# ykevinc/pocket-tts

Measured on AMD Instinct MI355X. Metric: audio-sec/wall-sec (RTF) per GPU at batch=32 + p50 first-chunk latency, higher is better.
Workload: dtype f32; 1 GPU; b6369a24 batch=32 concurrent 10 s utterances per GPU (125 frames, voice prompt 125 frames, 40 text tokens), lsd_decode_steps=1 (BASELINE configs[2]); global_batch=32, utterance_frames=125, jobs=37, prompt_frames=125, parallelism=replicas x1

## Files before the change

pocket-tts_amd/csrc/engine.cpp:

```cpp
#include "engine.h"

#include <hip/hip_ext.h>

#include <algorithm>
#include <array>
#include <cstdlib>
#include <cmath>
#include <cstring>
#include <mutex>

namespace ptts {

namespace {
std::mutex& voice_mu() {
  static std::mutex m;
  return m;
}

int pick_splits(int M, int N, int K) {
  const int tiles = ((N + 31) / 32) * ((M + 31) / 32);
  const int chunks = K / 32;
  int s = std::max(1, 768 / std::max(1, tiles));
  s = std::min(s, std::max(1, chunks / 4));
  return std::min(s, 16);
// ... 48 lines not shown
  PTTS_REQUIRE(!(cfg.fp8_gemm && cfg.weight_quant != QUANT_NONE), "fp8_gemm and weight_quant are exclusive");
  fp8_ = cfg.fp8_gemm;
  PTTS_REQUIRE(cfg.back_frames >= 0 && cfg.back_frames <= NFR_MAX && !(cfg.back_frames & (cfg.back_frames - 1)),
               "back_frames must be 0, 1, 2, 4 or 8");
  nfr_ = cfg.pipeline && cfg.back_frames >= 2 ? cfg.back_frames : 1;
  PTTS_REQUIRE(cfg.back_mfma >= PTTS_BACK_F32 && cfg.back_mfma <= PTTS_BACK_F32X6, "unknown back_mfma mode");
  back_mfma_ = cfg.back_mfma;
  nhb_ = nfr_ > 1 ? 3 * nfr_ : 3;
  int ndev = 0;
  PTTS_HIP(hipGetDeviceCount(&ndev));
  PTTS_REQUIRE(dev_ >= 0 && dev_ < ndev, "HIP device ordinal out of range");
  PTTS_HIP(hipSetDevice(dev_));
  PTTS_HIP(hipStreamCreateWithFlags(&stream_, hipStreamNonBlocking));

  L_ = pack_weights(nullptr, nullptr);
  if (cfg.weight_blob) {
    blob_ = (float*)cfg.weight_blob;
    own_blob_ = false;
  } else {
    blob_ = dalloc(L_.total);
  }

  const int B = max_slots_;
  kv_layer_ = (long)2 * NH * max_ctx_ * 64;
  kv_slot_ = kv_layer_ * NL;
  kv_ = dalloc((size_t)kv_slot_ * B);
  ring_layer_ = (long)2 * MNH * RING * 64;
  ring_slot_ = ring_layer_ * MNL;
  ring_ = dalloc((size_t)ring_slot_ * B);
  fpos_ = (int*)dalloc(B);
  mpos_ = (int*)dalloc(B);
  st_ = (SlotState*)dalloc((sizeof(SlotState) * B + 3) / 4);
  lat_in_ = dalloc((size_t)B * LDIM);
  cur_ = dalloc((size_t)B * LDIM);
  qprev_ = dalloc((size_t)(1 + NFR_MAX) * B * MD);
  qcur_ = qprev_ + (size_t)B * MD;
  eos_ = dalloc(B);
  static_assert(sizeof(FrameFlags) == 2 * sizeof(float), "FrameFlags packs into two floats");
  meta_floats_ = (size_t)B * (LDIM + 1 + 2);
  const size_t mstride = (meta_floats_ + 31) / 32 * 32;
  if (nfr_ > 1)
    for (int p = 0; p < nhb_ / nfr_; ++p) {
      const size_t n = (size_t)B * nfr_ * FRAME + nfr_ * mstride;
      pcmp_[p] = dalloc(n);
      PTTS_HIP(hipHostMalloc((void**)&h_pcmp_[p], sizeof(float) * n, hipHostMallocDefault));
    }
  for (int q = 0; q < NHB; ++q) {
    meta_[q] = nfr_ > 1 && q < nhb_ ? pcmp_[q / nfr_] + (size_t)B * nfr_ * FRAME + (q % nfr_) * mstride
                                    : dalloc(meta_floats_);
    lat_out_[q] = meta_[q];
    flags_[q] = (FrameFlags*)(meta_[q] + (size_t)B * LDIM);
    eos_out_[q] = meta_[q] + (size_t)B * (LDIM + 2);
    pcm_[q] = dalloc((size_t)B * FRAME);
  }
  fin_side_ = dalloc((size_t)B * (nfr_ * FRAME / RESBLOCK_FIN_TT) * 2);
  PTTS_HIP(hipHostMalloc((void**)&h_act_, sizeof(SlotState) * B, hipHostMallocDefault));
  mpcap_ = (size_t)nfr_ * std::max({(size_t)8 * B * UP * MD, (size_t)4 * B * UP * RATIOS[0] * (MD / 2)});
  mpartial_ = dalloc(mpcap_);

  const int hT[8] = {16, 16, 96, 96, 480, 480, 1920, 1920};
  const int hC[8] = {512, 512, 256, 256, 128, 128, 64, 64};
  const int hP[8] = {6, 1, 2, 1, 2, 1, 2, 2};
  for (int i = 0; i < 8; ++i) {
    hist_T_[i] = hT[i];
    hist_C_[i] = hC[i];
    hist_P_[i] = hP[i];
    hist_[i] = dalloc((size_t)B * hP[i] * hC[i]);
  }

  const int R = std::max(B, PREFILL);
  x_ = dalloc((size_t)R * D);
  h_ = dalloc((size_t)R * D);
  q_ = dalloc((size_t)R * D);
  o_ = dalloc((size_t)R * D);
  u_ = dalloc((size_t)R * FF);
  pcap_ = std::max({(size_t)4 << 20, (size_t)2 * B * UP * 3 * MD, (size_t)PREFILL * FF});
  partial_ = dalloc(pcap_);
  tslab_ = dalloc(TAIL_CAP);
  tickets_ = (int*)dalloc(TICKETS);
  fbm_.x = x_, fbm_.h = h_, fbm_.q = q_, fbm_.o = o_, fbm_.u = u_, fbm_.partial = partial_;
  fbm_.pcap = pcap_, fbm_.tslab = tslab_, fbm_.tail_cap = (long)TAIL_CAP, fbm_.tickets = tickets_;
  fbm_.kv = KvStore{kv_, kv_slot_, max_ctx_};
  fbm_.kv_layer = kv_layer_;
  ids_dev_ = (int*)dalloc(PREFILL);
  rowtab_dev_ = (int*)dalloc(PREFILL);
  ctab_dev_ = (int*)dalloc(PREFILL);
  qrow_dev_ = (int*)dalloc(PREFILL);
  orow_dev_ = (int*)dalloc(PREFILL);
  admit_slots_ = (int*)dalloc(B);
  admit_st_ = (SlotState*)dalloc((sizeof(SlotState) * B + 3) / 4);
  admit_fpos_ = (int*)dalloc(B);
  vpre_ = (const float**)dalloc((sizeof(float*) * B + 3) / 4);
  vlen_ = (int*)dalloc(B);
  slot_voice_.assign(B, nullptr);
  drained_.assign(B, 1);
  admit_call_.assign(B, -1);
  slot_lsd_.assign(B, 0);
  share_voice_ = probe_env("PTTS_NO_SHARED_VOICE") == nullptr;
#ifdef PTTS_PROBES
  if (probe_env("PTTS_STAMPS")) {
    stamp_ring_ = (unsigned long long*)dalloc((size_t)STAMP_CAP * 4);
    stamp_ctr_ = (unsigned*)dalloc(1);
  }
#endif
  if (probe_env("PTTS_BACK_WG_CAP")) back_cap_ = atoi(probe_env("PTTS_BACK_WG_CAP"));
  if (probe_env("PTTS_FRONT_PRIO")) set_front_prio(atoi(probe_env("PTTS_FRONT_PRIO")));
  if (probe_env("PTTS_BACK_PRIO")) set_back_prio(atoi(probe_env("PTTS_BACK_PRIO")));
  if (probe_env("PTTS_FRONT_SKIP")) set_front_skip(atoi(probe_env("PTTS_FRONT_SKIP")));
  ysilu_ = dalloc((size_t)lsd_ * B * FD);
  mods_ = dalloc((size_t)lsd_ * B * NADA);
  xf_ = dalloc((size_t)B * FD);
  hf_ = dalloc((size_t)B * FD);
  uf_ = dalloc((size_t)B * FD);
  PTTS_REQUIRE(hx_floats(B) * 4 < (1ull << 31), "flow-head hand-off regions exceed 2 GB (lsd_decode_steps too large)");
  hx_ = dalloc(hx_floats(B));
  fhm_ = dalloc((size_t)lsd_ * ((B + 15) / 16) * (FDEPTH + 1) * 2 * 16 * FD);
  PTTS_HIP(hipMemset(hx_, 0xFF, hx_floats(B) * 4));
  PTTS_HIP(hipDeviceSynchronize());
  hctr_ = (int*)dalloc(4 * ((B + 15) / 16) + 4);
  herr_ = (int*)dalloc(4);
  const size_t BF = (size_t)B * nfr_;
  mx_ = dalloc(BF * UP * MD);
  mh_ = dalloc(BF * UP * MD);
  mq_ = dalloc(BF * UP * MD);
  mo_ = dalloc(BF * UP * MD);
  mqkv_ = dalloc(BF * UP * 3 * MD);
  mu_ = dalloc(BF * UP * MFF);
  a0_ = dalloc(BF * 16 * 512);
  int T = 16, ch = 512;
  for (int i = 0; i < 3; ++i) {
    T *= RATIOS[i];
    ch /= 2;
    cb_[i] = dalloc(BF * T * ch);
    ce_[i] = dalloc(BF * T * ch);
    cv_[i] = dalloc(BF * T * (ch / 2));
    ca_[i] = dalloc(BF * T * ch);
    trb_[i] = dalloc((size_t)RATIOS[i] * ch);
  }
  temb_ = dalloc((size_t)temb_row0(lsd_ + 1) * FD);
  rope_ = dalloc((size_t)max_ctx_ * 64);
  temb_tmp_ = dalloc((size_t)2 * lsd_ * FD);

  for (int q = 0; q < NHB; ++q) {
    PTTS_HIP(hipHostMalloc((void**)&h_pcm_[q], sizeof(float) * B * FRAME, hipHostMallocDefault));
    if (nfr_ > 1 && q < nhb_)
      h_meta_[q] = h_pcmp_[q / nfr_] + (size_t)B * nfr_ * FRAME + (q % nfr_) * ((meta_floats_ + 31) / 32 * 32);
    else
      PTTS_HIP(hipHostMalloc((void**)&h_meta_[q], sizeof(float) * meta_floats_, hipHostMallocDefault));
    memset(h_meta_[q], 0, sizeof(float) * meta_floats_);
  }
  PTTS_HIP(hipHostMalloc((void**)&h_err_, sizeof(int), hipHostMallocDefault));
  *h_err_ = 0;
  PTTS_HIP(hipHostMalloc((void**)&h_slots_, sizeof(int) * B, hipHostMallocDefault));
  PTTS_HIP(hipHostMalloc((void**)&h_st_, sizeof(SlotState) * B, hipHostMallocDefault));
  PTTS_HIP(hipHostMalloc((void**)&h_fp_, sizeof(int) * B, hipHostMallocDefault));
  PTTS_HIP(hipHostMalloc((void**)&h_ids_, sizeof(int) * PREFILL, hipHostMallocDefault));
  PTTS_HIP(hipHostMalloc((void**)&h_tab_, sizeof(int) * 4 * PREFILL, hipHostMallocDefault));
  PTTS_HIP(hipHostMalloc((void**)&h_vpre_, sizeof(float*) * B, hipHostMallocDefault));
  PTTS_HIP(hipHostMalloc((void**)&h_vlen_, sizeof(int) * B, hipHostMallocDefault));
  memset(h_vpre_, 0, sizeof(float*) * B);
  memset(h_vlen_, 0, sizeof(int) * B);
  PTTS_HIP(hipStreamCreateWithFlags(&stream_be_, hipStreamNonBlocking));
  for (int q = 0; q < NHB; ++q) {
    PTTS_HIP(hipEventCreateWithFlags(&ev_front_[q], hipEventDisableTiming));
    PTTS_HIP(hipEventCreateWithFlags(&ev_back_[q], hipEventDisableTiming));
    PTTS_HIP(hipEventRecord(ev_front_[q], stream_));
    PTTS_HIP(hipEventRecord(ev_back_[q], stream_));
  }
  PTTS_HIP(hipEventCreateWithFlags(&ev_admit_, hipEventDisableTiming));
  PTTS_HIP(hipEventCreateWithFlags(&ev_be_tail_, hipEventDisableTiming));
  PTTS_HIP(hipEventCreateWithFlags(&ev_act_, hipEventDisableTiming));
  for (hipEvent_t& e : ev_call_) PTTS_HIP(hipEventCreateWithFlags(&e, hipEventDisableTiming));
  PTTS_HIP(hipEventRecord(ev_act_, stream_));
  PTTS_HIP(hipEventRecord(ev_admit_, stream_));
  pipeline_ = cfg.pipeline != 0;
  head_resident_ = flow_head_max_resident(dev_);

  if (!cfg.defer_weights) {
    std::unique_ptr<TensorSource> src = cfg.weights_path && cfg.weights_path[0]
                                            ? make_safetensors_source(cfg.weights_path)
                                            : make_synth_source(cfg.synth_seed);
    src = make_quant_source(std::move(src), wq_);
    upload_weights(src.get());
    finalize();
  }
}

Engine::~Engine() {
  (void)hipSetDevice(dev_);
  if (stream_) (void)hipStreamSynchronize(stream_);
  if (stream_be_) (void)hipStreamSynchronize(stream_be_);
  if (stream_pv_) (void)hipStreamSynchronize(stream_pv_);
  if (stream_vc_) (void)hipStreamSynchronize(stream_vc_);
#ifdef PTTS_PROBES
  if (stamp_ring_) {
    unsigned n = 0;
    std::vector<unsigned long long> r((size_t)STAMP_CAP * 2);
    if (hipMemcpy(&n, stamp_ctr_, 4, hipMemcpyDeviceToHost) == hipSuccess &&
        hipMemcpy(r.data(), stamp_ring_, r.size() * 8, hipMemcpyDeviceToHost) == hipSuccess)
      if (FILE* f = fopen(probe_env("PTTS_STAMPS"), "w")) {
        for (int p = 0; p < 2; ++p)
          for (size_t i = 0; i < stamp_names_[p].size(); ++i) fprintf(f, "# %d %zu %s\n", p, i, stamp_names_[p][i].c_str());
        for (unsigned i = 0; i < std::min(n, STAMP_CAP); ++i) fprintf(f, "%llu %llu\n", r[2 * i], r[2 * i + 1]);
        fclose(f);
      }
  }
#endif
  for (int s = 0; s < (int)slot_voice_.size(); ++s) voice_release(s, true);
  for (auto& kv : graphs_) (void)hipGraphExecDestroy(kv.second);
  for (auto& kv : graph_defs_) (void)hipGraphDestroy(kv.second);
  for (auto& kv : pv_graphs_) (void)hipGraphExecDestroy(kv.second);
  for (auto& kv : pv_graph_defs_) (void)hipGraphDestroy(kv.second);
  for (PvEntry& q : pv_q_) {
    if (q.ev) (void)hipEventDestroy(q.ev);
    if (q.h_pcm) (void)hipHostFree(q.h_pcm);
  }
  for (int q = 0; q < NHB; ++q)
    if (ev_pv_read_[q]) (void)hipEventDestroy(ev_pv_read_[q]);
  if (ev_pv_front_) (void)hipEventDestroy(ev_pv_front_);
  if (stream_pv_) (void)hipStreamDestroy(stream_pv_);
  for (int q = 0; q < NHB; ++q) {
    if (ev_front_[q]) (void)hipEventDestroy(ev_front_[q]);
    if (ev_back_[q]) (void)hipEventDestroy(ev_back_[q]);
  }
  if (ev_admit_) (void)hipEventDestroy(ev_admit_);
  if (ev_be_tail_) (void)hipEventDestroy(ev_be_tail_);
  if (ev_act_) (void)hipEventDestroy(ev_act_);
  for (hipEvent_t e : ev_call_)
    if (e) (void)hipEventDestroy(e);
  if (stream_be_) (void)hipStreamDestroy(stream_be_);
  vws_free(vws_);
  for (hipEvent_t e : vws_.ev_up)
    if (e) (void)hipEventDestroy(e);
  if (stream_vc_) (void)hipStreamDestroy(stream_vc_);
  for (void* p : allocs_) (void)hipFree(p);
  for (int q = 0; q < NHB; ++q) {
    if (h_pcm_[q]) (void)hipHostFree(h_pcm_[q]);
    if (h_meta_[q] && !(nfr_ > 1 && q < nhb_)) (void)hipHostFree(h_meta_[q]);
  }
  for (int p = 0; p < NHB / 2; ++p)
    if (h_pcmp_[p]) (void)hipHostFree(h_pcmp_[p]);
  if (h_act_) (void)hipHostFree(h_act_);
  if (h_err_) (void)hipHostFree(h_err_);
  for (void* hp : {(void*)h_slots_, (void*)h_st_, (void*)h_fp_, (void*)h_ids_, (void*)h_tab_, (void*)h_vpre_,
                   (void*)h_vlen_})
    if (hp) (void)hipHostFree(hp);
  if (stream_) (void)hipStreamDestroy(stream_);
}

void Engine::upload_weights(TensorSource* src) {
  std::vector<float> host(L_.total, 0.f);
  pack_weights(src, host.data());
  PTTS_HIP(hipMemcpy(blob_, host.data(), host.size() * sizeof(float), hipMemcpyHostToDevice));
}

void Engine::load_blob(const float* host, size_t n_bytes) {
  PTTS_REQUIRE(n_bytes == L_.total * sizeof(float), "blob size differs from ptts_weight_blob_bytes()");
  PTTS_REQUIRE(!ready_, "engine already finalized");
  PTTS_HIP(hipSetDevice(dev_));
  PTTS_HIP(hipMemcpy(blob_, host, n_bytes, hipMemcpyHostToDevice));
}

const uint32_t* Engine::pack_codes(const float* W, int N, int K, int nj,
                                   const std::function<void(const float*, float*)>& pack) {
  auto it = q8map_.find(W);
  auto it8 = f8map_.find(W);
  if (it == q8map_.end() && it8 == f8map_.end()) return nullptr;
  const size_t n = (size_t)N * K;
  float* tmp = nullptr;
  PTTS_HIP(hipMalloc(&tmp, sizeof(float) * 2 * n));
  void* q = nullptr;
  PTTS_HIP(hipMalloc(&q, n));
  allocs_.push_back(q);
  if (it != q8map_.end()) codes_to_f32(it->second.first, (long)n, tmp, stream_);
  else codes_u8_to_f32(it8->second.first, (long)n, tmp, stream_);
  pack(tmp, tmp + n);
  pack_q8(tmp + n, (long)(n / 4), nj, (uint32_t*)q, stream_);
  PTTS_HIP(hipStreamSynchronize(stream_));
  PTTS_HIP(hipFree(tmp));
  return (const uint32_t*)q;
}

void Engine::derive_gemv() {
  int mask = pipeline_ && nfr_ == 1 ? 2 | 8 | 16 : 31;
  if (probe_env("PTTS_GEMV_MASK")) mask = atoi(probe_env("PTTS_GEMV_MASK"));
  gemv_mask_ = mask;
  struct M {
    const float* w;
    int N, K, bit;
    GemvShape g;
  };
  std::vector<M> mats;
  const GemvShape wide{4, 128};
  const GemvShape outg{1, 32};
  for (int l = 0; l < NL; ++l) {
    const Layout::TL& t = L_.fl[l];
    mats.push_back({W(t.in_proj), 3 * D, D, 1, wide});
    mats.push_back({W(t.out_proj), D, D, 2, outg});
    mats.push_back({W(t.l1), FF, D, 4, wide});
    mats.push_back({W(t.l2), D, FF, 8, GemvShape{1, 64}});
  }
  const GemvShape ada{4, 128};
  mats.push_back({W(L_.ada_w), NADA, FD, 16, ada});
  auto scale_of = [&](const float* w) { return fp8_ ? f8map_.at(w).second : q8map_.at(w).second; };
  if ((mask & 4) && !probe_env("PTTS_NO_FK") && gemv_fk_supported(1, FF, D)) {
    const bool ffn = !probe_env("PTTS_NO_FFN") && ffn_fused_supported(1, D, FF);
    if (ffn) ffn_groups_ = probe_env("PTTS_FFN16") ? 16 : 8;
    const int G = ffn_groups_;
    std::vector<std::pair<const uint32_t*, const uint32_t*>> codes(NL, {nullptr, nullptr});
    bool all_codes = ffn;
    for (int l = 0; l < NL && ffn; ++l) {
      const float *w1 = W(L_.fl[l].l1), *w2 = W(L_.fl[l].l2);
      codes[l].first = pack_codes(w1, FF, D, 8, [&](const float* c, float* o) { pack_gemv_fk(c, FF, D, o, stream_); });
      codes[l].second = pack_codes(w2, D, FF, 8, [&](const float* c, float* o) { pack_ffn2(c, G, o, stream_); });
      if (codes[l].first && codes[l].second) ffn8map_[w2] = {{codes[l].first, scale_of(w1)}, {codes[l].second, scale_of(w2)}};
      else all_codes = false;
    }
    const bool f32_copies = !all_codes;
    void* q = nullptr;
    PTTS_HIP(hipMalloc(&q, sizeof(float) * ((f32_copies ? (size_t)NL * FF * D : 0) + FK_A_FLOATS)));
    allocs_.push_back(q);
    float* dst = (float*)q;
    for (int l = 0; l < NL; ++l) {
      if (f32_copies) pack_gemv_fk(W(L_.fl[l].l1), FF, D, dst, stream_);
      fkmap_[W(L_.fl[l].l1)] = f32_copies ? dst : nullptr;
      if (f32_copies) dst += (size_t)FF * D;
    }
    hfrag_ = dst;
// ... 2013 lines not shown
    PTTS_HIP(hipStreamCreateWithPriority(&stream_vc_, hipStreamNonBlocking, least));
    for (hipEvent_t& e : vws_.ev_up) PTTS_HIP(hipEventCreateWithFlags(&e, hipEventDisableTiming));
  }
  vws_reserve(vws_, stream_vc_, std::max(frames, vws_.frames), host_bytes, up_bytes);
}

void Engine::voice_jobs_reserve(int max_frames) {
  PTTS_REQUIRE(ready_, "engine weights not finalized");
  PTTS_REQUIRE(max_frames >= 1 && max_frames < max_ctx_, "max_frames must be in [1, max_ctx)");
  const size_t up = al16((size_t)max_frames * FRAME * 2 * sizeof(float)) + (64 << 10);
  vjob_reserve(max_frames, up, up);
}

ptts_voice* Engine::voice_job_prompt(const float* prompt, int F) {
  PTTS_REQUIRE(ready_, "engine weights not finalized");
  PTTS_REQUIRE(prompt != nullptr && F >= 1, "empty prompt");
  PTTS_REQUIRE(F < max_ctx_, "prompt longer than max_ctx");
  return voice_job(nullptr, prompt, F);
}

ptts_voice* Engine::voice_job_audio(const void* samples, int n_in, int fmt, int sr, int chunk_frames, int resampler) {
  PTTS_REQUIRE(ready_, "engine weights not finalized");
  PTTS_REQUIRE(samples != nullptr, "empty PCM");
  const VoicePlan p = voice_plan(n_in, fmt, sr, chunk_frames, resampler, max_ctx_);
  return voice_job(&p, samples, p.F);
}

void Engine::slot_open(int slot, const ptts_voice* v, const int32_t* ids, int n, const ptts_gen_params& p,
                       int lsd_steps) {
  slots_open(1, &slot, &v, ids, &n, &p, &lsd_steps);
}

int Engine::lsd_run_for(int B) const {
  int run = 0;
  for (int b = 0; b < B; ++b)
    if (!drained_[b]) run = std::max(run, slot_lsd_[b]);
  return run > 0 ? run : lsd_;
}

void Engine::slots_open(int n, const int* slots, const ptts_voice* const* voices, const int32_t* ids,
                        const int* n_ids, const ptts_gen_params* params, const int* lsd_steps) {
  PTTS_REQUIRE(ready_, "engine weights not finalized");
  PTTS_REQUIRE(n >= 1 && n <= max_slots_, "number of admissions out of range");
  PTTS_REQUIRE(slots && voices && n_ids && params, "null argument");
  std::vector<char> seen(max_slots_, 0);
  long total_ids = 0;
  for (int i = 0; i < n; ++i) {
    const int slot = slots[i];
    PTTS_REQUIRE(slot >= 0 && slot < max_slots_, "slot out of range");
    PTTS_REQUIRE(!seen[slot], "slot admitted twice in one call");
    seen[slot] = 1;
    const ptts_voice* v = voices[i];
    PTTS_REQUIRE(v != nullptr && v->owner == this, "voice belongs to another engine");
    const ptts_gen_params& p = params[i];
    PTTS_REQUIRE(n_ids[i] >= 0 && (n_ids[i] == 0 || ids != nullptr), "bad token ids");
    PTTS_REQUIRE(p.max_frames >= 1, "max_frames must be >= 1");
    PTTS_REQUIRE(!lsd_steps || lsd_steps[i] == 0 || (lsd_steps[i] >= 1 && lsd_steps[i] <= lsd_),
                 "lsd_steps must be 0 (the default) or in [1, " + std::to_string(lsd_) + "] (the engine's lsd_decode_steps)");
    PTTS_REQUIRE(p.frames_after_eos >= 0, "frames_after_eos must be >= 0");
    PTTS_REQUIRE((long)v->F + n_ids[i] + p.max_frames <= max_ctx_, "voice + text + max_frames exceeds max_ctx");
    for (int j = 0; j < n_ids[i]; ++j)
      PTTS_REQUIRE(ids[total_ids + j] >= 0 && ids[total_ids + j] < VOCAB, "token id out of range");
    total_ids += n_ids[i];
  }
  PTTS_HIP(hipEventSynchronize(ev_admit_));
  PTTS_HIP(hipEventSynchronize(ev_act_));
  for (int i = 0; i < n; ++i) {
    const ptts_voice* v = voices[i];
    if (!v->ev || v->ordered) continue;
    if (hipEventQuery(v->ev) != hipSuccess) PTTS_HIP(hipStreamWaitEvent(stream_, v->ev, 0));
    v->ordered = true;
  }
  if (share_voice_) {
    {
      std::lock_guard<std::mutex> lk(voice_mu());
      for (int i = 0; i < n; ++i) ++voices[i]->refs;
    }
    for (int i = 0; i < n; ++i) voice_release(slots[i], false);
    for (int i = 0; i < n; ++i) {
      slot_voice_[slots[i]] = voices[i];
      h_vpre_[slots[i]] = voices[i]->kv;
      h_vlen_[slots[i]] = voices[i]->F;
    }
    PTTS_HIP(hipMemcpyAsync(vpre_, h_vpre_, sizeof(float*) * max_slots_, hipMemcpyHostToDevice, stream_));
    PTTS_HIP(hipMemcpyAsync(vlen_, h_vlen_, sizeof(int) * max_slots_, hipMemcpyHostToDevice, stream_));
  } else {
    for (int i = 0; i < n; ++i) {
      const ptts_voice* v = voices[i];
      PTTS_HIP(hipMemcpy2DAsync(kv_ + (size_t)slots[i] * kv_slot_, sizeof(float) * max_ctx_ * 64, v->kv,
                                sizeof(float) * v->F * 64, sizeof(float) * v->F * 64, NL * 2 * NH,
                                hipMemcpyDeviceToDevice, stream_));
    }
  }
  std::vector<int> tab, rid;
  long off = 0;
  for (int i = 0; i < n; ++i) {
    for (int j = 0; j < n_ids[i]; ++j) {
      tab.push_back(slots[i] << 16 | (voices[i]->F + j));
      rid.push_back(ids[off + j]);
    }
    while (tab.size() % 16) {
      tab.push_back(-1);
      rid.push_back(0);
    }
    off += n_ids[i];
  }
  for (size_t c0 = 0; c0 < tab.size(); c0 += PREFILL) {
    const int T = (int)std::min<size_t>(PREFILL, tab.size() - c0);
    if (c0 > 0) PTTS_HIP(hipStreamSynchronize(stream_));
    int* h_ptab = h_tab_;
    int* h_ctab = h_tab_ + PREFILL;
    int* h_qrow = h_tab_ + 2 * PREFILL;
    int* h_orow = h_tab_ + 3 * PREFILL;
    int Tc = 0;
    for (int r = 0; r < T; ++r) {
      const int v = tab[c0 + r];
      h_ptab[r] = v;
      h_orow[r] = v < 0 ? -1 : Tc;
      if (v >= 0) {
        h_ctab[Tc] = v;
        h_qrow[Tc] = r;
        h_ids_[Tc] = rid[c0 + r];
        ++Tc;
      }
    }
    if (Tc == 0) continue;
    PTTS_HIP(hipMemcpyAsync(ids_dev_, h_ids_, sizeof(int) * Tc, hipMemcpyHostToDevice, stream_));
    PTTS_HIP(hipMemcpyAsync(rowtab_dev_, h_ptab, sizeof(int) * T, hipMemcpyHostToDevice, stream_));
    PTTS_HIP(hipMemcpyAsync(ctab_dev_, h_ctab, sizeof(int) * Tc, hipMemcpyHostToDevice, stream_));
    PTTS_HIP(hipMemcpyAsync(qrow_dev_, h_qrow, sizeof(int) * Tc, hipMemcpyHostToDevice, stream_));
    PTTS_HIP(hipMemcpyAsync(orow_dev_, h_orow, sizeof(int) * T, hipMemcpyHostToDevice, stream_));
    std::vector<Op> ops;
    {
      const int* idp = ids_dev_;
      const float* tb = W(L_.embed);
      float* x = x_;
      ops.push_back({"prefill.embed", [=](hipStream_t s) { embed_gather(idp, Tc, tb, D, x, s); }});
    }
    {
      float* x = x_;
      float* h = h_;
      const float* w = W(L_.fl[0].n1w);
      const float* b = W(L_.fl[0].n1b);
      ops.push_back({"prefill.ln1", [=](hipStream_t s) { layernorm(x, D, h, D, Tc, D, w, b, 1e-5f, s); }});
    }
    RowMap map{0, 1, 0, nullptr, ctab_dev_};
    map.ptab = rowtab_dev_;
    map.mpad = T;
    map.qrow = qrow_dev_;
    map.orow = orow_dev_;
    flow_layers(ops, Tc, map, 16, false, "prefill");
    run_ops(ops);
  }
  bool drained = true;
  for (int i = 0; i < n; ++i) drained = drained && drained_[slots[i]];
  if (!drained) {
    PTTS_HIP(hipEventRecord(ev_be_tail_, stream_be_));
    PTTS_HIP(hipStreamWaitEvent(stream_, ev_be_tail_, 0));
  }
  for (int i = 0; i < n; ++i) {
    drained_[slots[i]] = 0;
    admit_call_[slots[i]] = k_;
    slot_lsd_[slots[i]] = lsd_steps && lsd_steps[i] ? lsd_steps[i] : lsd_;
  }
  std::vector<SlotState> st(n);
  std::vector<int> fp(n);
  for (int i = 0; i < n; ++i) {
    const ptts_gen_params& p = params[i];
    SlotState& s = st[i];
    s = SlotState{};
    s.active = 1;
    s.step = 0;
    s.eos_step = -1;
    s.frames_after_eos = p.frames_after_eos;
    s.max_frames = p.max_frames;
    s.temp = p.temp;
    s.eos_threshold = p.eos_threshold;
    s.noise_clamp = p.noise_clamp;
    s.seed = p.seed;
    s.lsd = slot_lsd_[slots[i]];
    fp[i] = voices[i]->F + n_ids[i];
  }
  admit_delay_ = nfr_ > 1 ? (int)((nfr_ - k_ % nfr_) % nfr_) : 0;
  if (admit_delay_)
    for (int i = 0; i < n; ++i) {
      h_act_[slots[i]] = st[i];
      act_slots_.push_back(slots[i]);
      st[i].active = 0;
    }
  for (int i = 0; i < n; ++i) pv_forget(slots[i]);
  if (pv_max_ > 0)
    for (int i = 0; i < n; ++i) pv_pending_.push_back({slots[i], k_ + admit_delay_});
  memcpy(h_slots_, slots, sizeof(int) * n);
  memcpy(h_st_, st.data(), sizeof(SlotState) * n);
  memcpy(h_fp_, fp.data(), sizeof(int) * n);
  PTTS_HIP(hipMemcpyAsync(admit_slots_, h_slots_, sizeof(int) * n, hipMemcpyHostToDevice, stream_));
  PTTS_HIP(hipMemcpyAsync(admit_st_, h_st_, sizeof(SlotState) * n, hipMemcpyHostToDevice, stream_));
  PTTS_HIP(hipMemcpyAsync(admit_fpos_, h_fp_, sizeof(int) * n, hipMemcpyHostToDevice, stream_));
  {
    ResetArgs r{};
    for (int i = 0; i < 8; ++i) {
      r.buf[i] = hist_[i];
      r.per_slot[i] = (long)hist_P_[i] * hist_C_[i];
    }
    r.buf[8] = qprev_;
    r.per_slot[8] = MD;
    r.nb = 9;
    r.slots = admit_slots_;
    r.n = n;
    r.lat_in = lat_in_;
    r.bos = W(L_.bos);
    r.st_src = admit_st_;
    r.fpos_src = admit_fpos_;
    r.st = st_;
    r.fpos = fpos_;
    r.mpos = mpos_;
    for (int q = 0; q < NHB; ++q) r.flags[q] = flags_[q];
    slot_reset(r, stream_);
    PTTS_HIP(hipGetLastError());
  }
  mark_admission();
  admitted_since_call_ = true;
}

void Engine::mark_admission() {
  PTTS_HIP(hipEventRecord(ev_admit_, stream_));
  admit_pending_ = true;
  xh_dirty_ = true;
}

void Engine::refresh_xh() {
  input_ln(lat_in_, inw_t_, W(L_.fl[0].n1w), W(L_.fl[0].n1b), x_, h_, max_slots_, stream_);
  PTTS_HIP(hipGetLastError());
  xh_dirty_ = false;
}

void Engine::decode_latents(int slot, const float* lat, int n, float* pcm, float* quant, float* up, float* tr) {
  PTTS_REQUIRE(ready_, "engine weights not finalized");
  PTTS_REQUIRE(slot >= 0 && slot < max_slots_, "slot out of range");
  PTTS_REQUIRE(lat != nullptr && n >= 1, "no latents");
  sync();
  for (int q = 0; q < NHB; ++q) PTTS_HIP(hipMemsetAsync(flags_[q], 0, sizeof(FrameFlags) * max_slots_, stream_));
  {
    SlotState s{};
    s.eos_step = -1;
    *h_slots_ = slot;
    *h_st_ = s;
    *h_fp_ = 0;
    PTTS_HIP(hipMemcpyAsync(admit_slots_, h_slots_, sizeof(int), hipMemcpyHostToDevice, stream_));
    PTTS_HIP(hipMemcpyAsync(admit_st_, h_st_, sizeof(SlotState), hipMemcpyHostToDevice, stream_));
    PTTS_HIP(hipMemcpyAsync(admit_fpos_, h_fp_, sizeof(int), hipMemcpyHostToDevice, stream_));
    ResetArgs r{};
    for (int i = 0; i < 8; ++i) {
      r.buf[i] = hist_[i];
      r.per_slot[i] = (long)hist_P_[i] * hist_C_[i];
    }
    r.buf[8] = qprev_;
    r.per_slot[8] = MD;
    r.nb = 9;
    r.slots = admit_slots_;
    r.n = 1;
    r.lat_in = lat_in_;
    r.bos = W(L_.bos);
    r.st_src = admit_st_;
    r.fpos_src = admit_fpos_;
    r.st = st_;
    r.fpos = fpos_;
    r.mpos = mpos_;
    for (int q = 0; q < NHB; ++q) r.flags[q] = flags_[q];
    slot_reset(r, stream_);
    PTTS_HIP(hipGetLastError());
  }
  const FrameFlags on{1, 0}, off{0, 0};
  auto rows16 = [&](float* dst, const float* src) {
    PTTS_HIP(hipMemcpyAsync(dst, src + (size_t)slot * UP * MD, sizeof(float) * UP * MD, hipMemcpyDeviceToHost,
                            stream_));
  };
  for (int i = 0; i < n; ++i) {
    const int par = i & 1;
    PTTS_HIP(hipMemcpyAsync(lat_out_[par] + (size_t)slot * LDIM, lat + (size_t)i * LDIM, sizeof(float) * LDIM,
                            hipMemcpyHostToDevice, stream_));
    PTTS_HIP(hipMemcpyAsync(flags_[par] + slot, &on, sizeof on, hipMemcpyHostToDevice, stream_));
    std::vector<Op> ops;
    build_back(ops, slot + 1, par, 1, par, 1);
    size_t j = 0;
    for (; j < ops.size(); ++j) {
      if (ops[j].name == "seanet.conv0" && tr) rows16(tr + (size_t)i * UP * MD, mx_);
      ops[j].fn(stream_);
      hipError_t e = hipGetLastError();
      if (e != hipSuccess) throw Error(PTTS_ERR_HIP, "launch of " + ops[j].name + " failed: " + hipGetErrorString(e));
      if (j == 0 && up) rows16(up + (size_t)i * UP * MD, mx_);
    }
    if (pcm)
      PTTS_HIP(hipMemcpyAsync(pcm + (size_t)i * FRAME, pcm_[par] + (size_t)slot * FRAME, sizeof(float) * FRAME,
                              hipMemcpyDeviceToHost, stream_));
    if (quant)
      PTTS_HIP(hipMemcpyAsync(quant + (size_t)i * MD, qcur_ + (size_t)slot * NFR_MAX * MD,
                              sizeof(float) * MD, hipMemcpyDeviceToHost, stream_));
    PTTS_HIP(hipMemcpyAsync(flags_[par] + slot, &off, sizeof off, hipMemcpyHostToDevice, stream_));
    PTTS_HIP(hipStreamSynchronize(stream_));
  }
  mark_admission();
  drained_[slot] = 1;
  pv_forget(slot);
}

void Engine::slot_close(int slot) {
  PTTS_REQUIRE(slot >= 0 && slot < max_slots_, "slot out of range");
  sync();
  act_slots_.erase(std::remove(act_slots_.begin(), act_slots_.end(), slot), act_slots_.end());
  SlotState s{};
  s.eos_step = -1;
  memcpy(h_st_, &s, sizeof s);
  PTTS_HIP(hipMemcpyAsync(st_ + slot, h_st_, sizeof s, hipMemcpyHostToDevice, stream_));
  for (int q = 0; q < NHB; ++q)
    PTTS_HIP(hipMemsetAsync(flags_[q] + slot, 0, sizeof(FrameFlags), stream_));
  if (share_voice_ && slot_voice_[slot]) {
    h_vpre_[slot] = nullptr;
    h_vlen_[slot] = 0;
    PTTS_HIP(hipMemcpyAsync(vpre_ + slot, h_vpre_ + slot, sizeof(float*), hipMemcpyHostToDevice, stream_));
    PTTS_HIP(hipMemcpyAsync(vlen_ + slot, h_vlen_ + slot, sizeof(int), hipMemcpyHostToDevice, stream_));
  }
  mark_admission();
  PTTS_HIP(hipStreamSynchronize(stream_));
  drained_[slot] = 1;
  pv_forget(slot);
  voice_release(slot, true);
}

void Engine::voice_release(int slot, bool drained) {
  const ptts_voice* v = slot_voice_[slot];
  if (!v) return;
  slot_voice_[slot] = nullptr;
  bool free_now = false;
// ... 210 lines not shown
```

pocket-tts_amd/csrc/engine.h:

```cpp
#pragma once
#include <functional>
#include <map>
#include <string>
#include <vector>

#include "common.h"
#include "kernels.h"
#include "weights.h"

struct ptts_voice {
  int F = 0;
  float* kv = nullptr;
  std::vector<float> cond;
  const void* owner = nullptr;
  mutable int refs = 0;
  mutable bool dead = false;
  hipEvent_t ev = nullptr;
  float* h_cond = nullptr;
  mutable bool ordered = false;
};

namespace ptts {

struct VoicePlan;
// ... 62 lines not shown
  float* dalloc(size_t n);
  const float* W(size_t off) const { return blob_ + off; }
  void upload_weights(TensorSource* src);
  void derive_int8();
  void derive_fp8();
  struct FlowBufs {
    float *x = nullptr, *h = nullptr, *q = nullptr, *o = nullptr, *u = nullptr, *partial = nullptr;
    size_t pcap = 0;
    float* tslab = nullptr;
    long tail_cap = 0;
    int* tickets = nullptr;
    KvStore kv{};
    long kv_layer = 0;
  };
  FlowBufs fbm_{};
  void prefill_rows(std::vector<Op>& ops, int slot, int T, int p0, const FlowBufs* fb = nullptr);
  void run_ops(const std::vector<Op>& ops);
  void run_ops_on(const std::vector<Op>& ops, hipStream_t s);
  std::vector<Op> build_step(int B);
  void build_front(std::vector<Op>& ops, int B, int hb, int lsd_run);
  void build_back(std::vector<Op>& ops, int B, int hb, int nfr, int qp, int pcm_frames);
  hipGraphExec_t part_graph(int part, int B, int hb, int qp, int nfr, int lsd_run = 0);
  void wait_unless_done(hipStream_t s, hipEvent_t e);
  void copy_out(int B, int hb, hipStream_t s);
  void push_rr(std::vector<Op>& ops, const std::string& name, const RowReduceArgs& r);
  void flow_layers(std::vector<Op>& ops, int M, RowMap map, int qg, bool out_norm, const std::string& tag,
                   const FlowBufs* fb = nullptr);
  void linear_split(std::vector<Op>& ops, const std::string& name, const float* X, long ldx, int M, const float* Wt,
                    int N, int K, int* S_out, const FlowBufs* fb = nullptr);
  void conv_op(std::vector<Op>& ops, const std::string& name, const float* X, int B, int T_in, int cin, const float* H,
               int P, int stride, int elu, const float* Wt, int cout, int ktaps, int phases, const float* bias,
               const float* R, float* Y, int T_out, int tstride, int layout = 0, int elu_out = 0,
               float* Y2 = nullptr, int ksplit = 1);
  void dense_op(std::vector<Op>& ops, const std::string& name, const float* X, int M, const float* Wt, int N, int K,
                const float* bias, int act, const float* rscale, const float* R, float* Y,
                int layout = 0);
  void encoder_transformer(std::vector<Op>& ops, float* x, int T, float* h, float* qkv, float* q, float* o, float* u,
                           float* ring);

  static constexpr int LSD_MAX = 64;
  int dev_ = 0, max_slots_ = 0, max_ctx_ = 0, lsd_ = 1;
  std::vector<int> slot_lsd_;
  int lsd_last_run_ = 0;
  int lsd_run_for(int B) const;
  int wq_ = 0;
  std::map<const float*, std::pair<const int8_t*, const float*>> q8map_;
  int fp8_ = 0;
  std::map<const float*, std::pair<const uint8_t*, const float*>> f8map_;
  struct Gemv {
    const float* packed;
    GemvShape g;
    int bit;
    const uint32_t* q8;
    const float* scale;
  };
  const uint32_t* pack_codes(const float* W, int N, int K, int nj, const std::function<void(const float*, float*)>& pack);
  std::map<const float*, std::pair<std::pair<const uint32_t*, const float*>, std::pair<const uint32_t*, const float*>>>
      ffn8map_;
  std::map<const float*, Gemv> gvmap_;
  std::map<const float*, const float*> fkmap_;
  float* hfrag_ = nullptr;
  std::map<const float*, const float*> ffnmap_;
  float* ffn_hand_ = nullptr;
  int ffn_groups_ = 8;
  int gemv_mask_ = 0;
  void derive_gemv();
  bool own_blob_ = true, ready_ = false;
  hipStream_t stream_ = nullptr;
  Layout L_{};
  float* blob_ = nullptr;
  std::vector<void*> allocs_;

  float* kv_ = nullptr;
  long kv_slot_ = 0, kv_layer_ = 0;
  float* ring_ = nullptr;
  long ring_slot_ = 0, ring_layer_ = 0;
  int* fpos_ = nullptr;
  int* mpos_ = nullptr;
  bool share_voice_ = true;
  const float** vpre_ = nullptr;
  int* vlen_ = nullptr;
  const float** h_vpre_ = nullptr;
  int* h_vlen_ = nullptr;
  std::vector<const ptts_voice*> slot_voice_;
  void voice_release(int slot, bool drained);
  SlotState* st_ = nullptr;
  float *lat_in_ = nullptr, *cur_ = nullptr, *qprev_ = nullptr, *qcur_ = nullptr, *eos_ = nullptr;
  float* hist_[8] = {};
  int hist_T_[8] = {}, hist_C_[8] = {}, hist_P_[8] = {};

  static constexpr int PREFILL = 2048;
  size_t pcap_ = 0;
  float *x_ = nullptr, *h_ = nullptr, *q_ = nullptr, *o_ = nullptr, *u_ = nullptr, *partial_ = nullptr;
  static constexpr size_t TAIL_CAP = (size_t)16 << 20;
  static constexpr int TICKETS = 1024;
  float* tslab_ = nullptr;
  int* tickets_ = nullptr;
  int* ids_dev_ = nullptr;
  int* rowtab_dev_ = nullptr;
  int *ctab_dev_ = nullptr, *qrow_dev_ = nullptr, *orow_dev_ = nullptr;
  int* admit_slots_ = nullptr;
  SlotState* admit_st_ = nullptr;
  int* admit_fpos_ = nullptr;
  float *ysilu_ = nullptr, *mods_ = nullptr, *xf_ = nullptr, *hf_ = nullptr, *uf_ = nullptr;
  bool head_uniform_stride() const;
  bool use_head_chain(int B) const;
  float* fhw_ = nullptr;
  float* hx_ = nullptr;
  float* fhm_ = nullptr;
  float* fh_inw_t_ = nullptr;
  size_t hx_floats(int B) const { return hx_floats(B, lsd_); }
  size_t hx_floats(int B, int lsd) const { return (size_t)lsd * 13 * ((B + 15) / 16 * 16) * FD; }
  float* inw_t_ = nullptr;
  int *hctr_ = nullptr, *herr_ = nullptr;
  float *mx_ = nullptr, *mh_ = nullptr, *mq_ = nullptr, *mo_ = nullptr, *mqkv_ = nullptr, *mu_ = nullptr;
  float* a0_ = nullptr;
  float *cb_[3] = {}, *cv_[3] = {}, *ca_[3] = {}, *ce_[3] = {};
  float* trb_[3] = {};
  static constexpr int NHB = NHB_MAX;
  int nhb_ = 3;
  int nfr_ = 1;
  int back_mfma_ = PTTS_BACK_F32;
  std::map<const float*, std::pair<const unsigned*, const unsigned short*>> split_;
  void derive_split();
  void attach_split(GemmArgs& a) const;
  int rows_hb_[NHB] = {};
  float* pcmp_[NHB / 2] = {};
  float* h_pcmp_[NHB / 2] = {};
  float* fin_side_ = nullptr;
  SlotState* h_act_ = nullptr;
  std::vector<int> act_slots_;
  int admit_delay_ = 0;
  double plan_ctx_ = 0, plan_win_ = 0, plan_kvu_ = 0;
  float* lat_out_[NHB] = {};
  float* eos_out_[NHB] = {};
  FrameFlags* flags_[NHB] = {};
  float* pcm_[NHB] = {};
  float* meta_[NHB] = {};
  size_t meta_floats_ = 0;
  float* mpartial_ = nullptr;
  size_t mpcap_ = 0;
  int back_cap_ = 1;
  bool pipeline_ = false;
  hipStream_t stream_be_ = nullptr;
  hipEvent_t ev_front_[NHB] = {}, ev_back_[NHB] = {};
  hipEvent_t ev_admit_ = nullptr;
  hipEvent_t ev_be_tail_ = nullptr;
  hipEvent_t ev_act_ = nullptr;
  bool admit_pending_ = false;
  void mark_admission();
  long long k_ = 0;
  int out_hb_ = 0;
  int out_rows_ = 0;
  int prev_hb_ = 0, prev_rows_ = 0;
  long long out_k_ = -1, prev_k_ = -1;
  std::vector<long long> admit_call_;
  int front_rows_ = 0;
  bool admitted_since_call_ = false;
  bool xh_dirty_ = true;
  void refresh_xh();
  void call_async(int B, bool front);
  float *temb_ = nullptr, *temb_tmp_ = nullptr;
  float* rope_ = nullptr;

  float* h_pcm_[NHB] = {};
  float* h_meta_[NHB] = {};
  int* h_err_ = nullptr;
#ifdef PTTS_PROBES
  unsigned long long* stamp_ring_ = nullptr;
  unsigned* stamp_ctr_ = nullptr;
  std::vector<std::string> stamp_names_[2];
#endif
  int head_resident_ = 0;
  int *h_slots_ = nullptr, *h_fp_ = nullptr, *h_ids_ = nullptr, *h_tab_ = nullptr;
  SlotState* h_st_ = nullptr;

  std::map<int, hipGraphExec_t> graphs_;
  std::map<int, hipGraph_t> graph_defs_;

  std::vector<char> drained_;

  static constexpr int PV_MAX = 8;
  static constexpr int PV_Q = 8;
  struct BackBufs {
    float *ring = nullptr, *qprev = nullptr, *qcur = nullptr, *mx = nullptr, *mh = nullptr, *mq = nullptr,
          *mo = nullptr, *mqkv = nullptr, *mu = nullptr, *a0 = nullptr, *mpartial = nullptr, *fin_side = nullptr;
// ... 58 lines not shown
```

Baseline: 5254 audio-sec/wall-sec.

## Coalesce admission host-to-device uploads and overlap prefill tables on side stream

Packs the prefill index tables, the admission state arrays and the voice pointer/length tables into single contiguous pinned-host and device slabs. Each group then goes up in one memcpy instead of three to five separate small copies. When admitted slots are not yet drained, the prefill table upload is issued on a new upload stream and joined to the main stream with an event. The aim is to overlap it with back-end work rather than queue it behind it. Each copy now moves the full fixed-size slab, which is more bytes than before, and there is an added event/stream dependency to keep correct.

```diff
diff --git a/pocket-tts_amd/csrc/engine.cpp b/pocket-tts_amd/csrc/engine.cpp
--- a/pocket-tts_amd/csrc/engine.cpp
+++ b/pocket-tts_amd/csrc/engine.cpp
@@ -154,16 +154,18 @@
   fbm_.pcap = pcap_, fbm_.tslab = tslab_, fbm_.tail_cap = (long)TAIL_CAP, fbm_.tickets = tickets_;
   fbm_.kv = KvStore{kv_, kv_slot_, max_ctx_};
   fbm_.kv_layer = kv_layer_;
-  ids_dev_ = (int*)dalloc(PREFILL);
-  rowtab_dev_ = (int*)dalloc(PREFILL);
-  ctab_dev_ = (int*)dalloc(PREFILL);
-  qrow_dev_ = (int*)dalloc(PREFILL);
-  orow_dev_ = (int*)dalloc(PREFILL);
-  admit_slots_ = (int*)dalloc(B);
-  admit_st_ = (SlotState*)dalloc((sizeof(SlotState) * B + 3) / 4);
-  admit_fpos_ = (int*)dalloc(B);
-  vpre_ = (const float**)dalloc((sizeof(float*) * B + 3) / 4);
-  vlen_ = (int*)dalloc(B);
+  ids_dev_ = (int*)dalloc(5 * PREFILL);
+  rowtab_dev_ = ids_dev_ + PREFILL;
+  ctab_dev_ = ids_dev_ + 2 * PREFILL;
+  qrow_dev_ = ids_dev_ + 3 * PREFILL;
+  orow_dev_ = ids_dev_ + 4 * PREFILL;
+  admit_bytes_ = (sizeof(SlotState) + 2 * sizeof(int)) * B;
+  admit_st_ = (SlotState*)dalloc((admit_bytes_ + 3) / 4);
+  admit_slots_ = (int*)(admit_st_ + B);
+  admit_fpos_ = admit_slots_ + B;
+  vtab_bytes_ = (sizeof(float*) + sizeof(int)) * B;
+  vpre_ = (const float**)dalloc((vtab_bytes_ + 3) / 4);
+  vlen_ = (int*)(vpre_ + B);
   slot_voice_.assign(B, nullptr);
   drained_.assign(B, 1);
   admit_call_.assign(B, -1);
@@ -223,15 +225,18 @@
   }
   PTTS_HIP(hipHostMalloc((void**)&h_err_, sizeof(int), hipHostMallocDefault));
   *h_err_ = 0;
-  PTTS_HIP(hipHostMalloc((void**)&h_slots_, sizeof(int) * B, hipHostMallocDefault));
-  PTTS_HIP(hipHostMalloc((void**)&h_st_, sizeof(SlotState) * B, hipHostMallocDefault));
-  PTTS_HIP(hipHostMalloc((void**)&h_fp_, sizeof(int) * B, hipHostMallocDefault));
-  PTTS_HIP(hipHostMalloc((void**)&h_ids_, sizeof(int) * PREFILL, hipHostMallocDefault));
-  PTTS_HIP(hipHostMalloc((void**)&h_tab_, sizeof(int) * 4 * PREFILL, hipHostMallocDefault));
-  PTTS_HIP(hipHostMalloc((void**)&h_vpre_, sizeof(float*) * B, hipHostMallocDefault));
-  PTTS_HIP(hipHostMalloc((void**)&h_vlen_, sizeof(int) * B, hipHostMallocDefault));
-  memset(h_vpre_, 0, sizeof(float*) * B);
-  memset(h_vlen_, 0, sizeof(int) * B);
+  PTTS_HIP(hipHostMalloc((void**)&h_st_, admit_bytes_, hipHostMallocDefault));
+  memset(h_st_, 0, admit_bytes_);
+  h_slots_ = (int*)(h_st_ + B);
+  h_fp_ = h_slots_ + B;
+  PTTS_HIP(hipHostMalloc((void**)&h_ids_, sizeof(int) * 5 * PREFILL, hipHostMallocDefault));
+  memset(h_ids_, 0, sizeof(int) * 5 * PREFILL);
+  h_tab_ = h_ids_ + PREFILL;
+  PTTS_HIP(hipHostMalloc((void**)&h_vpre_, vtab_bytes_, hipHostMallocDefault));
+  memset(h_vpre_, 0, vtab_bytes_);
+  h_vlen_ = (int*)(h_vpre_ + B);
+  PTTS_HIP(hipStreamCreateWithFlags(&stream_up_, hipStreamNonBlocking));
+  PTTS_HIP(hipEventCreateWithFlags(&ev_up_, hipEventDisableTiming));
   PTTS_HIP(hipStreamCreateWithFlags(&stream_be_, hipStreamNonBlocking));
   for (int q = 0; q < NHB; ++q) {
     PTTS_HIP(hipEventCreateWithFlags(&ev_front_[q], hipEventDisableTiming));
@@ -264,6 +269,7 @@
   if (stream_be_) (void)hipStreamSynchronize(stream_be_);
   if (stream_pv_) (void)hipStreamSynchronize(stream_pv_);
   if (stream_vc_) (void)hipStreamSynchronize(stream_vc_);
+  if (stream_up_) (void)hipStreamSynchronize(stream_up_);
 #ifdef PTTS_PROBES
   if (stamp_ring_) {
     unsigned n = 0;
@@ -305,6 +311,8 @@
   for (hipEvent_t e : vws_.ev_up)
     if (e) (void)hipEventDestroy(e);
   if (stream_vc_) (void)hipStreamDestroy(stream_vc_);
+  if (ev_up_) (void)hipEventDestroy(ev_up_);
+  if (stream_up_) (void)hipStreamDestroy(stream_up_);
   for (void* p : allocs_) (void)hipFree(p);
   for (int q = 0; q < NHB; ++q) {
     if (h_pcm_[q]) (void)hipHostFree(h_pcm_[q]);
@@ -314,8 +322,7 @@
     if (h_pcmp_[p]) (void)hipHostFree(h_pcmp_[p]);
   if (h_act_) (void)hipHostFree(h_act_);
   if (h_err_) (void)hipHostFree(h_err_);
-  for (void* hp : {(void*)h_slots_, (void*)h_st_, (void*)h_fp_, (void*)h_ids_, (void*)h_tab_, (void*)h_vpre_,
-                   (void*)h_vlen_})
+  for (void* hp : {(void*)h_st_, (void*)h_ids_, (void*)h_vpre_})
     if (hp) (void)hipHostFree(hp);
   if (stream_) (void)hipStreamDestroy(stream_);
 }
@@ -2495,8 +2502,7 @@
       h_vpre_[slots[i]] = voices[i]->kv;
       h_vlen_[slots[i]] = voices[i]->F;
     }
-    PTTS_HIP(hipMemcpyAsync(vpre_, h_vpre_, sizeof(float*) * max_slots_, hipMemcpyHostToDevice, stream_));
-    PTTS_HIP(hipMemcpyAsync(vlen_, h_vlen_, sizeof(int) * max_slots_, hipMemcpyHostToDevice, stream_));
+    PTTS_HIP(hipMemcpyAsync(vpre_, h_vpre_, vtab_bytes_, hipMemcpyHostToDevice, stream_));
   } else {
     for (int i = 0; i < n; ++i) {
       const ptts_voice* v = voices[i];
@@ -2505,6 +2511,9 @@
                                 hipMemcpyDeviceToDevice, stream_));
     }
   }
+  bool drained = true;
+  for (int i = 0; i < n; ++i) drained = drained && drained_[slots[i]];
+  const bool early = !drained;
   std::vector<int> tab, rid;
   long off = 0;
   for (int i = 0; i < n; ++i) {
@@ -2538,11 +2547,12 @@
       }
     }
     if (Tc == 0) continue;
-    PTTS_HIP(hipMemcpyAsync(ids_dev_, h_ids_, sizeof(int) * Tc, hipMemcpyHostToDevice, stream_));
-    PTTS_HIP(hipMemcpyAsync(rowtab_dev_, h_ptab, sizeof(int) * T, hipMemcpyHostToDevice, stream_));
-    PTTS_HIP(hipMemcpyAsync(ctab_dev_, h_ctab, sizeof(int) * Tc, hipMemcpyHostToDevice, stream_));
-    PTTS_HIP(hipMemcpyAsync(qrow_dev_, h_qrow, sizeof(int) * Tc, hipMemcpyHostToDevice, stream_));
-    PTTS_HIP(hipMemcpyAsync(orow_dev_, h_orow, sizeof(int) * T, hipMemcpyHostToDevice, stream_));
+    PTTS_HIP(hipMemcpyAsync(ids_dev_, h_ids_, sizeof(int) * 5 * PREFILL, hipMemcpyHostToDevice,
+                            early ? stream_up_ : stream_));
+    if (early) {
+      PTTS_HIP(hipEventRecord(ev_up_, stream_up_));
+      PTTS_HIP(hipStreamWaitEvent(stream_, ev_up_, 0));
+    }
     std::vector<Op> ops;
     {
       const int* idp = ids_dev_;
@@ -2565,8 +2575,6 @@
     flow_layers(ops, Tc, map, 16, false, "prefill");
     run_ops(ops);
   }
-  bool drained = true;
-  for (int i = 0; i < n; ++i) drained = drained && drained_[slots[i]];
   if (!drained) {
     PTTS_HIP(hipEventRecord(ev_be_tail_, stream_be_));
     PTTS_HIP(hipStreamWaitEvent(stream_, ev_be_tail_, 0));
@@ -2607,9 +2615,7 @@
   memcpy(h_slots_, slots, sizeof(int) * n);
   memcpy(h_st_, st.data(), sizeof(SlotState) * n);
   memcpy(h_fp_, fp.data(), sizeof(int) * n);
-  PTTS_HIP(hipMemcpyAsync(admit_slots_, h_slots_, sizeof(int) * n, hipMemcpyHostToDevice, stream_));
-  PTTS_HIP(hipMemcpyAsync(admit_st_, h_st_, sizeof(SlotState) * n, hipMemcpyHostToDevice, stream_));
-  PTTS_HIP(hipMemcpyAsync(admit_fpos_, h_fp_, sizeof(int) * n, hipMemcpyHostToDevice, stream_));
+  upload_admit_state();
   {
     ResetArgs r{};
     for (int i = 0; i < 8; ++i) {
@@ -2636,6 +2642,10 @@
   admitted_since_call_ = true;
 }
 
+void Engine::upload_admit_state() {
+  PTTS_HIP(hipMemcpyAsync(admit_st_, h_st_, admit_bytes_, hipMemcpyHostToDevice, stream_));
+}
+
 void Engine::mark_admission() {
   PTTS_HIP(hipEventRecord(ev_admit_, stream_));
   admit_pending_ = true;
@@ -2660,9 +2670,7 @@
     *h_slots_ = slot;
     *h_st_ = s;
     *h_fp_ = 0;
-    PTTS_HIP(hipMemcpyAsync(admit_slots_, h_slots_, sizeof(int), hipMemcpyHostToDevice, stream_));
-    PTTS_HIP(hipMemcpyAsync(admit_st_, h_st_, sizeof(SlotState), hipMemcpyHostToDevice, stream_));
-    PTTS_HIP(hipMemcpyAsync(admit_fpos_, h_fp_, sizeof(int), hipMemcpyHostToDevice, stream_));
+    upload_admit_state();
     ResetArgs r{};
     for (int i = 0; i < 8; ++i) {
       r.buf[i] = hist_[i];
diff --git a/pocket-tts_amd/csrc/engine.h b/pocket-tts_amd/csrc/engine.h
--- a/pocket-tts_amd/csrc/engine.h
+++ b/pocket-tts_amd/csrc/engine.h
@@ -168,6 +168,7 @@
   int* vlen_ = nullptr;
   const float** h_vpre_ = nullptr;
   int* h_vlen_ = nullptr;
+  size_t vtab_bytes_ = 0;
   std::vector<const ptts_voice*> slot_voice_;
   void voice_release(int slot, bool drained);
   SlotState* st_ = nullptr;
@@ -188,6 +189,10 @@
   int* admit_slots_ = nullptr;
   SlotState* admit_st_ = nullptr;
   int* admit_fpos_ = nullptr;
+  size_t admit_bytes_ = 0;
+  void upload_admit_state();
+  hipStream_t stream_up_ = nullptr;
+  hipEvent_t ev_up_ = nullptr;
   float *ysilu_ = nullptr, *mods_ = nullptr, *xf_ = nullptr, *hf_ = nullptr, *uf_ = nullptr;
   bool head_uniform_stride() const;
   bool use_head_chain(int B) const;
```

Result: no change. 5242 audio-sec/wall-sec (-0.2%).
